# ICLDisco/ompi

Measured on AMD Instinct MI355X. Metric: Allreduce busBW GB/s @256MiB fp32 SUM at 2/4/8 GPUs; MPI_Op HBM GB/s, higher is better.
Workload: dtype f32; 1 GPU; MPI_Op 3-buffer SUM fp32, 1 GiB per buffer (BASELINE configs[1]); count=268435456, bytes_per_buffer=1073741824, op=MPI_SUM, datatype=MPI_FLOAT, kernel=op_vec_kernel<float,SUM,3buff>

## Files before the change

### ompi_amd/csrc/coll_ipc.hip

```cpp
#include <hip/hip_runtime.h>

#include <sched.h>
#include <unistd.h>

#include <algorithm>
#include <array>
#include <atomic>
#include <chrono>
#include <cstdarg>
#include <cstdio>
#include <cstdlib>
#include <cstring>
#include <deque>
#include <map>
#include <memory>
#include <mutex>
#include <new>
#include <utility>
#include <vector>

#include "../../include/ompi_amd_coll.h"
#include "bootstrap.h"
#include "comm_internal.h"
#include "host_mark.h"
#include "coll_kernels.h"
#include "coll_landing.h"
#include "ipc_registry.h"
#include "op_device.h"
#include "runtime.h"

namespace ompi_amd {

#define TRY(x)                                   \
    do {                                         \
        int rc_ = (x);                           \
        if (rc_ != OMPI_AMD_SUCCESS) return rc_; \
    } while (0)

__global__ void abort_kernel(flag_set peers, uint64_t *local, int rank, int size) {
    const int t = threadIdx.x;
    if (t < size && t != rank)
        __hip_atomic_store(peers.p[t] + kAbortWord, (uint64_t)1, __ATOMIC_RELAXED,
                           __HIP_MEMORY_SCOPE_SYSTEM);
    if (t == rank)
        __hip_atomic_store(local + kAbortWord, (uint64_t)1, __ATOMIC_RELAXED,
                           __HIP_MEMORY_SCOPE_SYSTEM);
    sys_release();
}

__global__ __launch_bounds__(64) void barrier_kernel(uint64_t *local, flag_set peers, int rank,
                                                     int size, uint64_t epoch, int *err,
                                                     uint64_t timeout_ticks, uint64_t *dbg) {
    const int t = threadIdx.x;
    if (dbg && t == 0)
        __hip_atomic_store(dbg, epoch, __ATOMIC_RELAXED, __HIP_MEMORY_SCOPE_SYSTEM);
    sys_release();
    if (t < size && t != rank)
        __hip_atomic_store(peers.p[t] + rank, epoch, __ATOMIC_RELAXED, __HIP_MEMORY_SCOPE_SYSTEM);
    if (t < size && t != rank)
        (void)wait_epoch(local + t, epoch, err, timeout_ticks, local + kAbortWord,
                         dbg ? dbg + 2 + t : nullptr);
    __syncthreads();
    sys_acquire();
    if (dbg && t == 0)
        __hip_atomic_store(dbg + 1, epoch, __ATOMIC_RELAXED, __HIP_MEMORY_SCOPE_SYSTEM);
}

__global__ void peek_kernel(const uint64_t *src, uint64_t *dst) {
    *dst = __hip_atomic_load(src, __ATOMIC_RELAXED, __HIP_MEMORY_SCOPE_SYSTEM);
}

struct tok_set { uint64_t t[kMaxRanks]; };
struct tok_ptrs { const uint64_t *p[kMaxRanks]; };
__global__ void land_stamp_kernel(uint64_t *mine, uint64_t token) {
    __hip_atomic_store(mine, token, __ATOMIC_RELAXED, __HIP_MEMORY_SCOPE_SYSTEM);
    sys_release();
}
__global__ __launch_bounds__(64) void land_check_kernel(tok_ptrs peers, tok_set expect, int rank, int size,
                                                        int *err, uint64_t *abort_word) {
    const int t = threadIdx.x;
    sys_acquire();
    if (t >= size || t == rank) return;
    if (__hip_atomic_load(peers.p[t], __ATOMIC_RELAXED, __HIP_MEMORY_SCOPE_SYSTEM) != expect.t[t]) {
        __hip_atomic_store(err, (int)OMPI_AMD_ERR_HIP, __ATOMIC_RELAXED, __HIP_MEMORY_SCOPE_SYSTEM);
        __hip_atomic_store(abort_word, (uint64_t)1, __ATOMIC_RELAXED, __HIP_MEMORY_SCOPE_SYSTEM);
    }
}

template <bool NT>
__global__ __launch_bounds__(kXferThreads) void copy_kernel(cp_jobs jobs) {
    acquire_once();
    const cp_job jb = jobs.j[blockIdx.y];
    const int64_t gstride = (int64_t)gridDim.x * kXferThreads;
    const int64_t tid = (int64_t)blockIdx.x * kXferThreads + threadIdx.x;
    const uintptr_t phase = (uintptr_t)jb.src ^ (uintptr_t)jb.dst;
    const int g = (phase & 15) == 0 ? 16 : ((phase & 3) == 0 ? 4 : 1);
    int64_t head = (int64_t)((g - ((uintptr_t)jb.src & (uintptr_t)(g - 1))) & (uintptr_t)(g - 1));
    if (head > jb.bytes) head = jb.bytes;
    const int64_t nbody = (jb.bytes - head) / g;
    const char *sb = jb.src + head;
    char *db = jb.dst + head;
    if (g == 16) {
        const u32x4 *s = reinterpret_cast<const u32x4 *>(sb);
        u32x4 *d = reinterpret_cast<u32x4 *>(db);
        int64_t i = tid;
        for (; i + 3 * gstride < nbody; i += 4 * gstride) {
            const u32x4 a = __builtin_nontemporal_load(s + i);
            const u32x4 b = __builtin_nontemporal_load(s + i + gstride);
            const u32x4 c = __builtin_nontemporal_load(s + i + 2 * gstride);
            const u32x4 e = __builtin_nontemporal_load(s + i + 3 * gstride);
            if constexpr (NT) {
                __builtin_nontemporal_store(a, d + i);
                __builtin_nontemporal_store(b, d + i + gstride);
                __builtin_nontemporal_store(c, d + i + 2 * gstride);
                __builtin_nontemporal_store(e, d + i + 3 * gstride);
            } else {
                d[i] = a;
                d[i + gstride] = b;
                d[i + 2 * gstride] = c;
                d[i + 3 * gstride] = e;
            }
        }
        for (; i < nbody; i += gstride) {
            if constexpr (NT) __builtin_nontemporal_store(__builtin_nontemporal_load(s + i), d + i);
            else d[i] = __builtin_nontemporal_load(s + i);
        }
    } else if (g == 4) {
        const uint32_t *s = reinterpret_cast<const uint32_t *>(sb);
        uint32_t *d = reinterpret_cast<uint32_t *>(db);
        for (int64_t i = tid; i < nbody; i += gstride) d[i] = s[i];
    } else {
        for (int64_t i = tid; i < nbody; i += gstride) db[i] = sb[i];
    }
    const int64_t tail0 = head + nbody * g;
    const int64_t nrest = head + (jb.bytes - tail0);
    for (int64_t k = tid; k < nrest; k += gstride) {
        const int64_t i = k < head ? k : tail0 + (k - head);
        jb.dst[i] = jb.src[i];
    }
    xfer_epilogue();
}

static red_launch_fn red_fn(int op, int type) {
    if (type < 0 || type >= OMPI_AMD_TYPE_COUNT) return nullptr;
    switch (op) {
#define CASE(k) case k: return red_row_##k()[type];
        OMPI_AMD_COLL_OPS(CASE)
#undef CASE
    default: return nullptr;
    }
}
static pipe_launch_fn pipe_fn(int op, int type) {
    if (type < 0 || type >= OMPI_AMD_TYPE_COUNT) return nullptr;
    switch (op) {
#define CASE(k) case k: return pipe_row_##k()[type];
        OMPI_AMD_COLL_OPS(CASE)
#undef CASE
    default: return nullptr;
    }
}
static fused_launch_fn fused_fn(int op, int type) {
    if (type < 0 || type >= OMPI_AMD_TYPE_COUNT) return nullptr;
    switch (op) {
#define CASE(k) case k: return fused_row_##k()[type];
        OMPI_AMD_COLL_OPS(CASE)
#undef CASE
    default: return nullptr;
    }
}

static size_t type_size(int type) {
    switch (type) {
    case OMPI_AMD_TYPE_DOUBLE_INT: case OMPI_AMD_TYPE_LONG_INT: return 12;
    case OMPI_AMD_TYPE_SHORT_INT: return 6;
    default: return ompi_amd_type_extent(type);
    }
}

static void blockcount(int64_t count, int n, int64_t *split, int64_t *early, int64_t *late) {
    *early = *late = count / n;
    *split = count % n;
    if (*split) *early += 1;
}
static int64_t block_off(int64_t b, int64_t split, int64_t early, int64_t late) {
    return b < split ? b * early : b * late + split;
}
static int64_t block_cnt(int64_t b, int64_t split, int64_t early, int64_t late) {
    return b < split ? early : late;
}

struct red_order { int order, first, flags; };
enum { TUNED_RED_LINEAR = 1, TUNED_RED_PIPELINE = 3, TUNED_RED_BINARY = 4, TUNED_RED_BINOMIAL = 5 };
enum { TUNED_RS_NONOVERLAPPING = 1, TUNED_RS_HALVING = 2, TUNED_RS_RING = 3 };
enum { TUNED_RSB_BASIC_LINEAR = 1 };
static bool tuned_red_alg_ok(int64_t v) {
    return v == 0 || v == TUNED_RED_LINEAR || v == TUNED_RED_PIPELINE || v == TUNED_RED_BINARY ||
           v == TUNED_RED_BINOMIAL;
}

static red_order tuned_reduce_order(int n, size_t msg, size_t count, int root, bool root_inplace,
                                    int forced = 0) {
    const int flr = root_inplace ? FOLD_ROOT_INPLACE : 0;
    switch (forced) {
    case TUNED_RED_LINEAR: return {ORDER_CHAIN, 0, 0};
    case TUNED_RED_PIPELINE: return {ORDER_CHAIN, root, flr};
    case TUNED_RED_BINARY: return {ORDER_BINARY, root, flr};
    case TUNED_RED_BINOMIAL: return {ORDER_BINOMIAL, root, flr};
    default: break;
    }
    const double a1 = 0.6016 / 1024.0, b1 = 1.3496;
    const double a2 = 0.0410 / 1024.0, b2 = 9.7128;
    const double a3 = 0.0422 / 1024.0, b3 = 1.1614;
    const int fl = root_inplace ? FOLD_ROOT_INPLACE : 0;
    const double m = (double)msg;
    if (n < 8 && msg < 512) return {ORDER_CHAIN, 0, 0};
    if ((n < 8 && msg < 20480) || msg < 2048 || count <= 1) return {ORDER_BINOMIAL, root, fl};
    if (n > a1 * m + b1) return {ORDER_BINOMIAL, root, fl};
    if (n > a2 * m + b2) return {ORDER_CHAIN, root, fl};
    if (n > a3 * m + b3) return {ORDER_BINARY, root, fl};
    return {ORDER_CHAIN, root, fl};
}

struct buf_desc {
    hipIpcMemHandle_t h;
    uint64_t off;
    uint64_t valid;
    uint64_t id;
    uint64_t base;
    uint64_t size;
    uint64_t pid;
};
struct call_blob {
    buf_desc s, r;
    uint64_t flags;
};
struct land_blob {
    buf_desc d;
    uint64_t token;
    int ok;
};

struct fold_plan {
    int order;
    int first;
    int flags;
};
enum {
    TUNED_AR_FIXED = 0, TUNED_AR_BASIC_LINEAR = 1, TUNED_AR_NONOVERLAPPING = 2,
    TUNED_AR_RECURSIVE_DOUBLING = 3, TUNED_AR_RING = 4, TUNED_AR_RING_SEGMENTED = 5,
    TUNED_AR_RABENSEIFNER = 6, TUNED_AR_COUNT = 7
};

struct path_params {
    size_t small_bytes, fused_bytes;
    int zero_copy, algorithm;
    int tuned_alg;
    int root0_inplace;
    int push_gather;
    int blocks = 0;
    int copy_nt = -1;
    int red_alg = 0;
};

struct shadow_set {
    cp_jobs in{};
    cp_job out{};
    char *mem = nullptr;
    char *mem2 = nullptr;
};

enum { XCH_ALLTOALL = 0, XCH_ALLGATHERV = 1, XCH_GATHER = 2, XCH_SCATTER = 3 };
struct a2a_call {
    const char *sbuf;
    char *rbuf;
    bool inplace;
    int coll;
    uint8_t ph[kMaxRanks];
    size_t sc[kMaxRanks], sd[kMaxRanks], rc[kMaxRanks], rd[kMaxRanks];
};

struct pending_op {
    uint64_t ticket;
    const void *sbuf;
    void *rbuf;
    size_t count;
    int type, op;
    hipStream_t stream;
    path_params pp;
    ompi_amd_request *req;
    shadow_set sh;
    int kind = 0;
    int root = 0;
    bool inplace = false;
    bool exclusive = false;
    bool land = false;
    std::vector<size_t> rcounts;
    bool unposted = false;
    size_t blob_len = 0;
    union {
        call_blob call;
        land_blob land;
    } blob{};
    char *grow = nullptr;
    size_t grow_bytes = 0;
    uint64_t grow_token = 0;
    a2a_call a2a{};
    size_t a2a_M = 0;
    size_t a2a_chunk = 0;
};

enum { PEND_ALLREDUCE = 0, PEND_RSB = 1, PEND_ALLGATHER = 2, PEND_BCAST = 3, PEND_REDUCE = 4,
       PEND_SCAN = 5, PEND_RS = 6, PEND_GROW = 7, PEND_ALLTOALL = 8 };

}

using namespace ompi_amd;

struct ompi_amd_request {
    ~ompi_amd_request() { mark_word_put(mark); }
    ompi_amd_comm_t *c = nullptr;
    hipEvent_t ev = nullptr;
    hipStream_t stream = nullptr;
    bool launched = false;
    bool recorded = false;
    uint64_t *mark = nullptr;
    uint64_t mark_seq = 0;
    int rc = OMPI_AMD_SUCCESS;
    char *shadow = nullptr;
    char *shadow2 = nullptr;
    uint64_t embedded = 0;
    int done_slot = -1;
    unsigned polls = 0;
};

constexpr int kTuneGrid = 18, kTuneCands = 2 * kTuneGrid, kTuneRounds = 2,
              kTuneCalls = kTuneCands * kTuneRounds;
struct tune_cand {
    int algorithm, blocks, nt;
};
static const tune_cand kTune[kTuneCands] = {
    {2, 1024, 1}, {2, 512, 1}, {2, 256, 1}, {3, 1024, 1}, {3, 512, 1}, {3, 256, 1},
    {0, 1024, 1}, {0, 512, 1}, {0, 256, 1}, {4, 1024, 1}, {4, 512, 1}, {4, 256, 1},
    {5, 1024, 1}, {5, 512, 1}, {5, 256, 1}, {6, 1024, 1}, {6, 512, 1}, {6, 256, 1},
    {2, 1024, 0}, {2, 512, 0}, {2, 256, 0}, {3, 1024, 0}, {3, 512, 0}, {3, 256, 0},
    {0, 1024, 0}, {0, 512, 0}, {0, 256, 0}, {4, 1024, 0}, {4, 512, 0}, {4, 256, 0},
    {5, 1024, 0}, {5, 512, 0}, {5, 256, 0}, {6, 1024, 0}, {6, 512, 0}, {6, 256, 0}};
struct tune_bucket {
    int ncand = kTuneCands;
    int next = 0;
    bool done = false;
    int choice = 0;
    hipEvent_t ev[2 * kTuneCalls] = {};
    float worst_ms[kTuneCands] = {};
};

struct ompi_amd_comm {
    int rank = 0, size = 0, device = 0;
    ShmBoot boot;
    uint64_t *flags = nullptr;
    flag_set peer_flags{};
    char *scratch = nullptr;
    size_t scratch_bytes = 0;
    uint64_t stage_seq = 0;
    ptr_set peer_scratch{};
    char *land = nullptr;
    size_t land_bytes = 0;
    ptr_set peer_land{};
    ipc_ref *land_ref[kMaxRanks] = {};
    size_t land_planned = 0;
    std::vector<char *> land_retired;
    std::vector<ipc_ref *> land_ref_retired;
    bool land_failed = false;
    int unposted = 0;
    int64_t deferred_growths = 0;
    std::vector<uint64_t> land_tokens;
    int memcpy_token_mismatch = 0;
    int bcast_split = 0;
    size_t bcast_split_bytes = 4u << 20;
    int64_t exports_new = 0, imports_new = 0;
    int recycled_exports = 0;
    int64_t reused_exports = 0;
    int reuse_shadow = 1;
    int unsafe_exports = 0;
    int aged_exports = 0;
    std::mutex stream_mu;
    std::recursive_mutex api_mu;
    std::atomic<int> npending{0};
    bool has_stream = false;
    hipStream_t cur_stream = nullptr;
    int own_stream = 0;
    hipStream_t own = nullptr;
    bool cur_closed = false;
    std::vector<hipEvent_t> stream_evs;
    char *shadow = nullptr;
    size_t shadow_bytes = 0;
    char *shadow2 = nullptr;
    size_t shadow2_bytes = 0;
    struct arena_chunk {
        char *base;
        size_t size;
        std::map<size_t, size_t> free;
        std::map<size_t, size_t> used;
    };
    std::mutex arena_mu;
    std::vector<arena_chunk> arena;
    size_t arena_bytes = 0;
    int shadowed = 0;
    int force_shadow = 0;
    int win_shadow = 0;
    int win_separate = 1;
    int64_t shadow_windows = 0;
    int user_ipc = 0;
    int *err_host = nullptr, *err_dev = nullptr;
    uint64_t *dbg_host = nullptr, *dbg_dev = nullptr;
    uint64_t epoch = 0;
    uint64_t *fused_mark = nullptr;
    bool want_mark = false;
    uint64_t mark_embedded = 0;
    uint64_t *mark_word = nullptr;
    int mark_slot = 0;
    std::vector<int> done_free;
    int done_next = 1;
    size_t small_bytes = 1 << 20;
    size_t fused_bytes = 64 << 10;
    int zero_copy = 1;
    int64_t timeout_ms = 30000;
    int max_blocks = 1024;
    int64_t pipe_slice = 64 << 10;
    int pipe_passes = 1;
    uint64_t pipe_seq = 0;
    int colocated = 1;
    int algorithm = 2;
    int autotune = 0;
    std::map<int, struct tune_bucket> tune;
    int tune_last = 0;
    int tune_last_key = -1;
    int nb_tuned_alg = -1, nb_tuned_blocks = -1, nb_tuned_nt = -1;
    int64_t land_ag_bcast = 0;
    int land_blocking = 0;
    size_t alltoall_chunk = 0;
    int64_t alltoall_passes = 0;
    int64_t alltoall_paths[5] = {};
    int64_t gather_paths[5] = {};
// ... 4337 lines not shown
```

### ompi_amd/csrc/coll_kern.hip

```cpp
#include <hip/hip_runtime.h>

#include <algorithm>
#include <array>
#include <utility>

#include "coll_kernels.h"

#ifndef COLL_OP
#error "build with -DCOLL_OP=<op index>"
#endif

namespace ompi_amd {
namespace {

template <int OP, int TYPE>
hipError_t red_launch_slot(dim3 grid, const ptr_set &src, const ptr_set &dst, int ndst, int n,
                           int order, int flags, const red_jobs &jobs, hipStream_t s) {
    if constexpr (slot_supported(OP, TYPE)) {
        using T = typename type_of<TYPE>::type;
        if (n <= 8)
            hipLaunchKernelGGL((reduce_kernel<T, OP, 8>), grid, dim3(kXferThreads), 0, s, src, dst,
                               ndst, n, order, flags, jobs);
        else
            hipLaunchKernelGGL((reduce_kernel<T, OP, kMaxRanks>), grid, dim3(kXferThreads), 0, s,
                               src, dst, ndst, n, order, flags, jobs);
        return hipGetLastError();
    } else {
        return hipErrorInvalidValue;
    }
}

template <int OP, int TYPE>
hipError_t fused_launch_slot(dim3 grid, const fused_args &a, hipStream_t s) {
    if constexpr (slot_supported(OP, TYPE)) {
        using T = typename type_of<TYPE>::type;
        hipLaunchKernelGGL((fused_allreduce_kernel<T, OP>), grid, dim3(kXferThreads), 0, s, a);
        return hipGetLastError();
    } else {
        return hipErrorInvalidValue;
    }
}

template <int OP, int TYPE>
hipError_t pipe_launch_slot(unsigned groups, const pipe_args &a, hipStream_t s) {
    if constexpr (slot_supported(OP, TYPE)) {
        using T = typename type_of<TYPE>::type;
        if (a.n > 8) return hipErrorInvalidValue;
        static const int64_t cap = [] {
            int per_cu = 0, cus = 0, dev = 0;
            if (hipGetDevice(&dev) != hipSuccess ||
                hipOccupancyMaxActiveBlocksPerMultiprocessor(
                    &per_cu, reinterpret_cast<const void *>(&pipe_allreduce_kernel<T, OP, 8>),
                    kXferThreads, 0) != hipSuccess ||
                hipDeviceGetAttribute(&cus, hipDeviceAttributeMultiprocessorCount, dev) != hipSuccess) {
                (void)hipGetLastError();
                return (int64_t)64;
            }
            return std::max<int64_t>(1, (int64_t)per_cu * cus / 2);
        }();
        const int64_t fit = std::max<int64_t>(1, cap / std::max(1, a.colocated));
        const dim3 g((unsigned)std::min<int64_t>(groups, fit)), b(kXferThreads);
        hipLaunchKernelGGL((pipe_allreduce_kernel<T, OP, 8>), g, b, 0, s, a);
        return hipGetLastError();
    } else {
        return hipErrorInvalidValue;
    }
}

template <int OP, int... T>
constexpr std::array<red_launch_fn, OMPI_AMD_TYPE_COUNT> make_red_row(std::integer_sequence<int, T...>) {
    return {{(slot_supported(OP, T) ? &red_launch_slot<OP, T> : (red_launch_fn) nullptr)...}};
}
template <int OP, int... T>
constexpr std::array<fused_launch_fn, OMPI_AMD_TYPE_COUNT> make_fused_row(
    std::integer_sequence<int, T...>) {
    return {{(slot_supported(OP, T) ? &fused_launch_slot<OP, T> : (fused_launch_fn) nullptr)...}};
}

template <int OP, int... T>
constexpr std::array<pipe_launch_fn, OMPI_AMD_TYPE_COUNT> make_pipe_row(
    std::integer_sequence<int, T...>) {
    return {{(slot_supported(OP, T) ? &pipe_launch_slot<OP, T> : (pipe_launch_fn) nullptr)...}};
}

const auto g_red_row = make_red_row<COLL_OP>(std::make_integer_sequence<int, OMPI_AMD_TYPE_COUNT>{});
const auto g_fused_row = make_fused_row<COLL_OP>(std::make_integer_sequence<int, OMPI_AMD_TYPE_COUNT>{});
const auto g_pipe_row = make_pipe_row<COLL_OP>(std::make_integer_sequence<int, OMPI_AMD_TYPE_COUNT>{});

}

#define ROW_NAME2(a, b) a##b
#define ROW_NAME(a, b) ROW_NAME2(a, b)
const red_launch_fn *ROW_NAME(red_row_, COLL_OP)() { return g_red_row.data(); }
const fused_launch_fn *ROW_NAME(fused_row_, COLL_OP)() { return g_fused_row.data(); }
const pipe_launch_fn *ROW_NAME(pipe_row_, COLL_OP)() { return g_pipe_row.data(); }

}
```

### ompi_amd/csrc/coll_kernels.h

```cpp
#pragma once

#include <hip/hip_runtime.h>

#include <cstdint>

#include "../../include/ompi_amd_coll.h"
#include "op_device.h"

namespace ompi_amd {

constexpr int kMaxRanks = OMPI_AMD_MAX_RANKS;
constexpr int kXferThreads = 256;

struct ptr_set { const char *p[kMaxRanks]; };
struct flag_set { uint64_t *p[kMaxRanks]; };

enum order_t {
    ORDER_RING = 0,
    ORDER_TREE = 1,
    ORDER_CHAIN = 2,
    ORDER_BINOMIAL = 3,
    ORDER_BINARY = 4,
    ORDER_HALVING = 5,
    ORDER_RABEN = 6,
};
constexpr int FOLD_ROOT_INPLACE = 1;
constexpr int FOLD_NT_STORE = 1 << 16;

struct red_job {
    int64_t off, cnt, off_dst;
    int first;
    int head;
    int aux = 0;
};
struct red_jobs { red_job j[2 * kMaxRanks]; int n; };

struct cp_job { const char *src; char *dst; int64_t bytes; };
struct cp_jobs { cp_job j[kMaxRanks]; int n; };

__device__ __forceinline__ void sys_acquire() {
    __builtin_amdgcn_fence(__ATOMIC_ACQUIRE, "");
    asm volatile("s_waitcnt vmcnt(0)" ::: "memory");
}
__device__ __forceinline__ void sys_release() {
    __builtin_amdgcn_fence(__ATOMIC_RELEASE, "");
    asm volatile("s_waitcnt vmcnt(0)" ::: "memory");
}

__device__ __forceinline__ void acquire_once() {
    if (threadIdx.x == 0) sys_acquire();
    __syncthreads();
}

constexpr int kAbortWord = 512;
constexpr size_t kFlagPageBytes = 8192;

__device__ __forceinline__ bool wait_epoch(const uint64_t *flag, uint64_t epoch, int *err,
                                           uint64_t ticks, uint64_t *abort_word,
                                           uint64_t *seen = nullptr) {
    const uint64_t t0 = __builtin_amdgcn_s_memrealtime();
    uint64_t check = t0 + 100000;
    while (__hip_atomic_load(flag, __ATOMIC_RELAXED, __HIP_MEMORY_SCOPE_SYSTEM) < epoch) {
        __builtin_amdgcn_s_sleep(1);
        const uint64_t now = __builtin_amdgcn_s_memrealtime();
        if (now - t0 > ticks) {
            __hip_atomic_store(err, (int)OMPI_AMD_ERR_TIMEOUT, __ATOMIC_RELAXED,
                               __HIP_MEMORY_SCOPE_SYSTEM);
            __hip_atomic_store(abort_word, (uint64_t)1, __ATOMIC_RELAXED, __HIP_MEMORY_SCOPE_SYSTEM);
            return false;
        }
        if (now >= check) {
            if (seen)
                __hip_atomic_store(seen, __hip_atomic_load(flag, __ATOMIC_RELAXED, __HIP_MEMORY_SCOPE_SYSTEM),
                                   __ATOMIC_RELAXED, __HIP_MEMORY_SCOPE_SYSTEM);
            if (__hip_atomic_load(abort_word, __ATOMIC_RELAXED, __HIP_MEMORY_SCOPE_SYSTEM) != 0) {
                __hip_atomic_store(err, (int)OMPI_AMD_ERR_TIMEOUT, __ATOMIC_RELAXED,
                                   __HIP_MEMORY_SCOPE_SYSTEM);
                return false;
            }
            check = now + 100000;
        }
    }
    return true;
}

__device__ __forceinline__ void xfer_epilogue() {
    asm volatile("s_waitcnt vmcnt(0)" ::: "memory");
    __syncthreads();
    if (threadIdx.x == 0) sys_release();
}

template <typename T, int OP, int NM = kMaxRanks>
__device__ __forceinline__ T fold(const T (&v)[NM], int n, int order, int flags) {
    using F = opfn<OP, false>;
    const bool swap = (flags & FOLD_ROOT_INPLACE) != 0;
    if (order == ORDER_RING) {
        T acc = v[0];
#pragma unroll
        for (int j = 1; j < NM; ++j)
            if (j < n) acc = F::template f<T>(v[j], acc);
        return acc;
    }
    if (order == ORDER_CHAIN) {
        T acc = v[NM - 1];
#pragma unroll
        for (int j = NM - 1; j >= 0; --j) {
            if (j == n - 1) acc = v[j];
            else if (j < n - 1) acc = (j == 0 && swap) ? F::template f<T>(v[0], acc)
                                                       : F::template f<T>(acc, v[j]);
        }
        return acc;
    }
    if (order == ORDER_BINOMIAL) {
        T w[NM];
#pragma unroll
        for (int i = 0; i < NM; ++i) w[i] = v[i];
#pragma unroll
        for (int u = 0; u + 1 < NM; u += 2)
            if (u + 1 < n) w[u] = (u == 0 && swap) ? F::template f<T>(w[0], w[1])
                                                   : F::template f<T>(w[u + 1], w[u]);
#pragma unroll
        for (int m = 2; m < NM; m <<= 1) {
#pragma unroll
            for (int u = 0; u + m < NM; u += 2 * m)
                if (u + m < n) w[u] = F::template f<T>(w[u], w[u + m]);
        }
        return w[0];
    }
    if (order == ORDER_BINARY) {
        T w[NM];
#pragma unroll
        for (int i = 0; i < NM; ++i) w[i] = v[i];
#pragma unroll
        for (int s = NM - 1; s >= 0; --s) {
            int d = 1;
            while (2 * d <= s + 1) d *= 2;
            const int c0 = s + d, c1 = s + 2 * d;
            if (c0 < NM && c0 < n)
                w[s] = (s == 0 && swap) ? F::template f<T>(w[0], w[c0])
                                        : F::template f<T>(w[c0], w[s]);
            if (c1 < NM && c1 < n) w[s] = F::template f<T>(w[s], w[c1]);
        }
        return w[0];
    }
    if (order == ORDER_RABEN) {
        int adj = 1;
        while (adj * 2 <= n) adj *= 2;
        const int rem = n - adj;
        const int o = (flags >> 8) & 0xff;
        const bool right = (o & 1) != 0;
        T w[NM];
#pragma unroll
        for (int u = 0; u < NM; ++u) {
            if (2 * u + 1 < NM && u < rem)
                w[u] = right ? F::template f<T>(v[2 * u + 1], v[2 * u])
                             : F::template f<T>(v[2 * u], v[2 * u + 1]);
            else if (u < adj)
                w[u] = v[u + rem < NM ? u + rem : 0];
        }
#pragma unroll
        for (int m = 1; m < NM; m <<= 1) {
            if (m < adj) {
#pragma unroll
                for (int u = 0; u < NM; ++u)
                    if (u < adj && (u & m) == (o & m)) w[u] = F::template f<T>(w[u], w[u ^ m]);
            }
        }
        T r = w[0];
#pragma unroll
        for (int u = 1; u < NM; ++u)
            if (u == o) r = w[u];
        return r;
    }
    if (order == ORDER_HALVING) {
        int adj = 1;
        while (adj * 2 <= n) adj *= 2;
        const int remain = n - adj;
        const int tb = (flags >> 8) & 0xff;
        T w[NM];
#pragma unroll
        for (int u = 0; u < NM; ++u) {
            if (2 * u + 1 < NM && u < remain) w[u] = F::template f<T>(v[2 * u + 1], v[2 * u]);
            else if (u < adj) w[u] = v[u + remain];
        }
#pragma unroll
        for (int m = NM / 2; m >= 1; m >>= 1) {
            if (m < adj) {
#pragma unroll
                for (int u = 0; u < NM; ++u)
                    if (u < adj && (u & m) == (tb & m)) w[u] = F::template f<T>(w[u], w[u ^ m]);
            }
        }
        T r = w[0];
#pragma unroll
        for (int u = 1; u < NM; ++u)
            if (u == tb) r = w[u];
        return r;
    }
    int adj = 1;
    while (adj * 2 <= n) adj *= 2;
    const int extra = n - adj;
    T w[NM];
#pragma unroll
    for (int i = 0; i < NM; ++i) {
        if (i < extra) w[i] = F::template f<T>(v[2 * i + 1], v[2 * i]);
        else if (i < adj) w[i] = v[i + extra];
    }
#pragma unroll
    for (int len = NM; len > 1; len >>= 1) {
        if (len <= adj) {
#pragma unroll
            for (int i = 0; i < NM / 2; ++i)
                if (2 * i + 1 < len) w[i] = F::template f<T>(w[2 * i + 1], w[2 * i]);
        }
    }
    return w[0];
}

template <typename T, int NM = kMaxRanks>
__device__ __forceinline__ void gather_scalar(T (&v)[NM], const ptr_set &src, int n,
                                              int first, int64_t e) {
#pragma unroll
    for (int j = 0; j < NM; ++j) {
        if (j < n) {
            const int r = (first + j) % n;
            v[j] = reinterpret_cast<const T *>(src.p[r])[e];
        }
    }
}

template <typename T, int OP, int NM = kMaxRanks>
__global__ __launch_bounds__(kXferThreads) void reduce_kernel(ptr_set src, ptr_set dst, int ndst,
                                                              int n, int order, int flags,
                                                              red_jobs jobs) {
    acquire_once();
    const red_job jb = jobs.j[blockIdx.y];
    constexpr int E = 16 / sizeof(T);
    const int64_t gstride = (int64_t)gridDim.x * kXferThreads;
    const int64_t tid = (int64_t)blockIdx.x * kXferThreads + threadIdx.x;
    const int64_t head = jb.head < 0 ? jb.cnt : jb.head;
    const int64_t nvec = jb.head < 0 ? 0 : (jb.cnt - head) / E;
    for (int64_t i = tid; i < nvec; i += gstride) {
        vec16<T> v[NM];
#pragma unroll
        for (int j = 0; j < NM; ++j) {
            if (j < n) {
                const int r = (jb.first + j) % n;
                const u32x4 *p = reinterpret_cast<const u32x4 *>(
                    reinterpret_cast<const T *>(src.p[r]) + jb.off + head);
                v[j].v = __builtin_nontemporal_load(p + i);
            }
        }
        vec16<T> out;
#pragma unroll
        for (int e = 0; e < E; ++e) {
            T s[NM];
#pragma unroll
            for (int j = 0; j < NM; ++j) s[j] = v[j].e[e];
            out.e[e] = fold<T, OP, NM>(s, n, order, flags | jb.aux);
        }
        if (flags & FOLD_NT_STORE) {
#pragma unroll
            for (int k = 0; k < NM; ++k)
                if (k < ndst)
                    __builtin_nontemporal_store(
                        out.v, reinterpret_cast<u32x4 *>(reinterpret_cast<T *>(const_cast<char *>(dst.p[k])) +
                                                         jb.off_dst + head) + i);
        } else {
#pragma unroll
            for (int k = 0; k < NM; ++k)
                if (k < ndst)
                    reinterpret_cast<u32x4 *>(reinterpret_cast<T *>(const_cast<char *>(dst.p[k])) +
                                              jb.off_dst + head)[i] = out.v;
        }
    }
    const int64_t tail0 = head + nvec * E;
    const int64_t nscalar = head + (jb.cnt - tail0);
    for (int64_t k = tid; k < nscalar; k += gstride) {
        const int64_t e = k < head ? k : tail0 + (k - head);
        T s[NM];
        gather_scalar<T, NM>(s, src, n, jb.first, jb.off + e);
        const T r = fold<T, OP, NM>(s, n, order, flags | jb.aux);
#pragma unroll
        for (int d = 0; d < NM; ++d)
            if (d < ndst)
                store_elem<T>(reinterpret_cast<T *>(const_cast<char *>(dst.p[d])) + jb.off_dst + e,
                              r);
    }
    xfer_epilogue();
}

constexpr int kFusedMaxGroups = 4096 / (int)sizeof(uint64_t) / kMaxRanks;

struct fused_args {
    const char *src;
    char *dst, *mine;
    ptr_set peers;
    uint64_t *flags;
    flag_set peer_flags;
    int rank, n, order;
    int64_t count, split, early, late;
    uint64_t epoch, timeout_ticks;
    int *err;
    uint32_t *done;
    uint64_t *mark;
    uint64_t mark_v;
};

constexpr int kFusedDoneWord = 8192 / (int)sizeof(uint32_t);
constexpr int kFusedDoneStride = 64 / (int)sizeof(uint32_t);
constexpr int kFusedDoneSlots = (64 << 10) / 64 - 8192 / 64;

template <typename T, int OP>
__global__ __launch_bounds__(kXferThreads) void fused_allreduce_kernel(fused_args a) {
    const int t = threadIdx.x;
    const int g = blockIdx.y * gridDim.x + blockIdx.x;
    int64_t off = 0, cnt = a.count;
    int first = 0;
    if (a.order == ORDER_RING) {
        const int64_t b = blockIdx.y;
        off = b < a.split ? b * a.early : b * a.late + a.split;
        cnt = b < a.split ? a.early : a.late;
        first = (int)b;
    }
    const int64_t per = (cnt + gridDim.x - 1) / gridDim.x;
    const int64_t lo = off + min(cnt, per * (int64_t)blockIdx.x);
    const int64_t hi = off + min(cnt, per * (int64_t)(blockIdx.x + 1));
    const T *src = reinterpret_cast<const T *>(a.src);
    T *mine = reinterpret_cast<T *>(a.mine);
    for (int64_t e = lo + t; e < hi; e += kXferThreads) mine[e] = src[e];
    asm volatile("s_waitcnt vmcnt(0)" ::: "memory");
    __syncthreads();
    if (t == 0) sys_release();
    __syncthreads();
    __shared__ int gave_up;
    if (t == 0) gave_up = 0;
    __syncthreads();
    if (t < a.n && t != a.rank) {
        __hip_atomic_store(a.peer_flags.p[t] + g * kMaxRanks + a.rank, a.epoch, __ATOMIC_RELAXED,
                           __HIP_MEMORY_SCOPE_SYSTEM);
        if (!wait_epoch(a.flags + g * kMaxRanks + t, a.epoch, a.err, a.timeout_ticks,
                        a.flags + kAbortWord))
            gave_up = 1;
    }
    __syncthreads();
    if (gave_up) return;
    acquire_once();
    T *dst = reinterpret_cast<T *>(a.dst);
    for (int64_t e = lo + t; e < hi; e += kXferThreads) {
        T v[kMaxRanks];
        gather_scalar<T>(v, a.peers, a.n, first, e);
        store_elem<T>(dst + e, fold<T, OP>(v, a.n, a.order, 0));
    }
    if (a.mark) {
        asm volatile("s_waitcnt vmcnt(0)" ::: "memory");
        __syncthreads();
        if (t == 0) {
            __builtin_amdgcn_fence(__ATOMIC_RELEASE, "agent");
            const uint32_t total = gridDim.x * gridDim.y;
            if (__hip_atomic_fetch_add(a.done, 1u, __ATOMIC_ACQ_REL, __HIP_MEMORY_SCOPE_AGENT) == total - 1) {
                __hip_atomic_store(a.done, 0u, __ATOMIC_RELAXED, __HIP_MEMORY_SCOPE_AGENT);
                __hip_atomic_store(a.mark, a.mark_v, __ATOMIC_RELAXED, __HIP_MEMORY_SCOPE_SYSTEM);
            }
        }
    }
}

constexpr int kPipeMaxGroups = 1024;
constexpr size_t kPipeFlagOff = 64 << 10;
constexpr size_t kPipeFlagBytes = 2 * (size_t)kPipeMaxGroups * kMaxRanks * sizeof(uint64_t);

struct pipe_args {
    const char *src;
    ptr_set dst_c;
    ptr_set src_f;
    ptr_set dst_f;
    ptr_set src_g;
    char *rbuf;
    uint64_t *flags;
    flag_set peer_flags;
    int rank, n, mine, ndst, order, first, fold_flags, nt;
    int colocated;
    int64_t split, early, late;
    int64_t per, nslices;
    uint64_t seq, timeout_ticks;
    int *err;
    uint64_t *abort_word;
};

__device__ __forceinline__ size_t pipe_row(int phase, int w, int r) {
    return ((size_t)phase * kPipeMaxGroups + (size_t)w) * kMaxRanks + (size_t)r;
}

__device__ __forceinline__ void pipe_copy(const char *s, char *d, int64_t lo, int64_t hi, bool nt) {
    const int t = threadIdx.x;
    if (hi <= lo) return;
    int64_t head = hi - lo, nv = 0;
    if ((((uintptr_t)(s + lo) ^ (uintptr_t)(d + lo)) & 15) == 0) {
        head = min(hi - lo, (int64_t)((16 - ((uintptr_t)(s + lo) & 15)) & 15));
        nv = (hi - lo - head) / 16;
    }
    const u32x4 *sv = reinterpret_cast<const u32x4 *>(s + lo + head);
    u32x4 *dv = reinterpret_cast<u32x4 *>(d + lo + head);
    constexpr int S = kXferThreads;
    int64_t i = t;
    for (; i + 3 * S < nv; i += 4 * S) {
        const u32x4 a = __builtin_nontemporal_load(sv + i);
        const u32x4 b = __builtin_nontemporal_load(sv + i + S);
        const u32x4 c = __builtin_nontemporal_load(sv + i + 2 * S);
        const u32x4 e = __builtin_nontemporal_load(sv + i + 3 * S);
        if (nt) {
            __builtin_nontemporal_store(a, dv + i);
            __builtin_nontemporal_store(b, dv + i + S);
            __builtin_nontemporal_store(c, dv + i + 2 * S);
            __builtin_nontemporal_store(e, dv + i + 3 * S);
        } else {
            dv[i] = a;
            dv[i + S] = b;
            dv[i + 2 * S] = c;
            dv[i + 3 * S] = e;
        }
    }
    for (; i < nv; i += S) {
        if (nt) __builtin_nontemporal_store(__builtin_nontemporal_load(sv + i), dv + i);
        else dv[i] = __builtin_nontemporal_load(sv + i);
    }
    const int64_t tail0 = lo + head + nv * 16;
    const int64_t nrest = head + (hi - tail0);
    for (int64_t k = t; k < nrest; k += S) {
        const int64_t b = k < head ? lo + k : tail0 + (k - head);
        d[b] = s[b];
    }
}

template <typename T, int OP, int NM>
__device__ __forceinline__ void pipe_fold(const pipe_args &a, int64_t lo, int64_t hi) {
    constexpr int E = 16 / sizeof(T);
    const int t = threadIdx.x;
    if (hi <= lo) return;
    const uintptr_t ph = (uintptr_t)(a.dst_f.p[0] + lo * (int64_t)sizeof(T)) & 15;
    bool same = true;
#pragma unroll
    for (int j = 0; j < NM; ++j)
        if (j < a.n) same = same && (((uintptr_t)(a.src_f.p[j] + lo * (int64_t)sizeof(T)) & 15) == ph);
#pragma unroll
    for (int k = 1; k < NM; ++k)
        if (k < a.ndst) same = same && (((uintptr_t)(a.dst_f.p[k] + lo * (int64_t)sizeof(T)) & 15) == ph);
    const int64_t lead = (int64_t)((16 - ph) & 15);
    int64_t head = hi - lo, nv = 0;
    if (same && lead % (int64_t)sizeof(T) == 0) {
        head = min(hi - lo, lead / (int64_t)sizeof(T));
        nv = (hi - lo - head) / E;
    }
    const int64_t v0 = lo + head;
    for (int64_t i = t; i < nv; i += kXferThreads) {
        vec16<T> v[NM];
#pragma unroll
        for (int j = 0; j < NM; ++j) {
            if (j < a.n) {
                const int r = (a.first + j) % a.n;
                const u32x4 *p = reinterpret_cast<const u32x4 *>(reinterpret_cast<const T *>(a.src_f.p[r]) + v0);
                v[j].v = __builtin_nontemporal_load(p + i);
            }
        }
        vec16<T> out;
#pragma unroll
        for (int e = 0; e < E; ++e) {
            T s[NM];
#pragma unroll
            for (int j = 0; j < NM; ++j) s[j] = v[j].e[e];
            out.e[e] = fold<T, OP, NM>(s, a.n, a.order, a.fold_flags);
        }
#pragma unroll
        for (int k = 0; k < NM; ++k) {
            if (k < a.ndst) {
                u32x4 *q = reinterpret_cast<u32x4 *>(reinterpret_cast<T *>(const_cast<char *>(a.dst_f.p[k])) + v0) + i;
                if (a.nt) __builtin_nontemporal_store(out.v, q);
                else *q = out.v;
            }
        }
    }
    const int64_t tail0 = v0 + nv * E;
    const int64_t nrest = head + (hi - tail0);
    for (int64_t k = t; k < nrest; k += kXferThreads) {
        const int64_t e = k < head ? lo + k : tail0 + (k - head);
        T s[NM];
        gather_scalar<T, NM>(s, a.src_f, a.n, a.first, e);
        const T r = fold<T, OP, NM>(s, a.n, a.order, a.fold_flags);
#pragma unroll
        for (int d = 0; d < NM; ++d)
            if (d < a.ndst) store_elem<T>(reinterpret_cast<T *>(const_cast<char *>(a.dst_f.p[d])) + e, r);
    }
}

template <typename T, int OP, int NM>
__global__ __launch_bounds__(kXferThreads) void pipe_allreduce_kernel(pipe_args a) {
    const int t = threadIdx.x, w = blockIdx.x, G = gridDim.x;
    const int64_t P = (a.nslices - w + G - 1) / G;
    constexpr int64_t ext = sizeof(T);
    __shared__ int gave_up;
    if (t == 0) gave_up = 0;
    __syncthreads();
    for (int64_t p = 0; p < P + 2; ++p) {
        const bool doC = p < P, doF = p >= 1 && p <= P, doG = p >= 2;
        if (p >= 1) {
            if (t < a.n && t != a.rank) {
                bool ok = true;
                if (doF)
                    ok = wait_epoch(a.flags + pipe_row(0, w, t), a.seq + (uint64_t)p, a.err,
                                    a.timeout_ticks, a.abort_word);
                if (ok && doG)
                    ok = wait_epoch(a.flags + pipe_row(1, w, t), a.seq + (uint64_t)(p - 1), a.err,
                                    a.timeout_ticks, a.abort_word);
                if (!ok) gave_up = 1;
            }
            __syncthreads();
            if (gave_up) return;
            acquire_once();
        }
        if (doC) {
            const int64_t s = w + p * G;
#pragma unroll
            for (int b = 0; b < NM; ++b) {
                if (b >= a.n || !a.dst_c.p[b]) continue;
                const int64_t off = b < a.split ? b * a.early : b * a.late + a.split;
                const int64_t cnt = b < a.split ? a.early : a.late;
                const int64_t lo = off + min(cnt, s * a.per), hi = off + min(cnt, (s + 1) * a.per);
                pipe_copy(a.src, const_cast<char *>(a.dst_c.p[b]), lo * ext, hi * ext, a.nt);
            }
        }
        if (doF) {
            const int64_t s = w + (p - 1) * G;
            const int b = a.mine;
            const int64_t off = b < a.split ? b * a.early : b * a.late + a.split;
            const int64_t cnt = b < a.split ? a.early : a.late;
            pipe_fold<T, OP, NM>(a, off + min(cnt, s * a.per), off + min(cnt, (s + 1) * a.per));
        }
        if (doG) {
            const int64_t s = w + (p - 2) * G;
#pragma unroll
            for (int b = 0; b < NM; ++b) {
                if (b >= a.n || !a.src_g.p[b]) continue;
                const int64_t off = b < a.split ? b * a.early : b * a.late + a.split;
                const int64_t cnt = b < a.split ? a.early : a.late;
                const int64_t lo = off + min(cnt, s * a.per), hi = off + min(cnt, (s + 1) * a.per);
                pipe_copy(a.src_g.p[b], a.rbuf, lo * ext, hi * ext, a.nt);
            }
        }
        if (doC || doF) {
            asm volatile("s_waitcnt vmcnt(0)" ::: "memory");
            __syncthreads();
            if (t == 0) sys_release();
            __syncthreads();
            if (t < a.n && t != a.rank) {
                if (doC)
                    __hip_atomic_store(a.peer_flags.p[t] + pipe_row(0, w, a.rank), a.seq + (uint64_t)(p + 1),
                                       __ATOMIC_RELAXED, __HIP_MEMORY_SCOPE_SYSTEM);
                if (doF)
                    __hip_atomic_store(a.peer_flags.p[t] + pipe_row(1, w, a.rank), a.seq + (uint64_t)p,
                                       __ATOMIC_RELAXED, __HIP_MEMORY_SCOPE_SYSTEM);
            }
        }
    }
    xfer_epilogue();
}

struct a2a_args {
    const char *sbuf;
    char *rbuf, *mine;
    ptr_set peers;
    uint64_t *flags;
    flag_set peer_flags;
    int rank, n;
    int self_copy;
    int64_t slot;
    int64_t scount[kMaxRanks], sdispl[kMaxRanks], rcount[kMaxRanks], rdispl[kMaxRanks];
    uint8_t sphase[kMaxRanks], rphase[kMaxRanks];
    uint64_t epoch, timeout_ticks;
    int *err;
    uint32_t *done;
    uint64_t *mark;
    uint64_t mark_v;
};

__host__ __device__ __forceinline__ void a2a_slice(int64_t b, int g, int G, int64_t *lo, int64_t *hi) {
    const int64_t per = ((b + G - 1) / G + 15) & ~(int64_t)15;
    *lo = per * g < b ? per * g : b;
    *hi = per * (g + 1) < b ? per * (g + 1) : b;
}

// ... 172 lines not shown
```

Measured before the change: 6488 GB/s.

## Specialize reduce kernel by rank count, unroll loads, and widen fold blocks

```diff
diff --git a/ompi_amd/csrc/coll_ipc.hip b/ompi_amd/csrc/coll_ipc.hip
--- a/ompi_amd/csrc/coll_ipc.hip
+++ b/ompi_amd/csrc/coll_ipc.hip
@@ -85,60 +85,6 @@
         __hip_atomic_store(err, (int)OMPI_AMD_ERR_HIP, __ATOMIC_RELAXED, __HIP_MEMORY_SCOPE_SYSTEM);
         __hip_atomic_store(abort_word, (uint64_t)1, __ATOMIC_RELAXED, __HIP_MEMORY_SCOPE_SYSTEM);
     }
-}
-
-template <bool NT>
-__global__ __launch_bounds__(kXferThreads) void copy_kernel(cp_jobs jobs) {
-    acquire_once();
-    const cp_job jb = jobs.j[blockIdx.y];
-    const int64_t gstride = (int64_t)gridDim.x * kXferThreads;
-    const int64_t tid = (int64_t)blockIdx.x * kXferThreads + threadIdx.x;
-    const uintptr_t phase = (uintptr_t)jb.src ^ (uintptr_t)jb.dst;
-    const int g = (phase & 15) == 0 ? 16 : ((phase & 3) == 0 ? 4 : 1);
-    int64_t head = (int64_t)((g - ((uintptr_t)jb.src & (uintptr_t)(g - 1))) & (uintptr_t)(g - 1));
-    if (head > jb.bytes) head = jb.bytes;
-    const int64_t nbody = (jb.bytes - head) / g;
-    const char *sb = jb.src + head;
-    char *db = jb.dst + head;
-    if (g == 16) {
-        const u32x4 *s = reinterpret_cast<const u32x4 *>(sb);
-        u32x4 *d = reinterpret_cast<u32x4 *>(db);
-        int64_t i = tid;
-        for (; i + 3 * gstride < nbody; i += 4 * gstride) {
-            const u32x4 a = __builtin_nontemporal_load(s + i);
-            const u32x4 b = __builtin_nontemporal_load(s + i + gstride);
-            const u32x4 c = __builtin_nontemporal_load(s + i + 2 * gstride);
-            const u32x4 e = __builtin_nontemporal_load(s + i + 3 * gstride);
-            if constexpr (NT) {
-                __builtin_nontemporal_store(a, d + i);
-                __builtin_nontemporal_store(b, d + i + gstride);
-                __builtin_nontemporal_store(c, d + i + 2 * gstride);
-                __builtin_nontemporal_store(e, d + i + 3 * gstride);
-            } else {
-                d[i] = a;
-                d[i + gstride] = b;
-                d[i + 2 * gstride] = c;
-                d[i + 3 * gstride] = e;
-            }
-        }
-        for (; i < nbody; i += gstride) {
-            if constexpr (NT) __builtin_nontemporal_store(__builtin_nontemporal_load(s + i), d + i);
-            else d[i] = __builtin_nontemporal_load(s + i);
-        }
-    } else if (g == 4) {
-        const uint32_t *s = reinterpret_cast<const uint32_t *>(sb);
-        uint32_t *d = reinterpret_cast<uint32_t *>(db);
-        for (int64_t i = tid; i < nbody; i += gstride) d[i] = s[i];
-    } else {
-        for (int64_t i = tid; i < nbody; i += gstride) db[i] = sb[i];
-    }
-    const int64_t tail0 = head + nbody * g;
-    const int64_t nrest = head + (jb.bytes - tail0);
-    for (int64_t k = tid; k < nrest; k += gstride) {
-        const int64_t i = k < head ? k : tail0 + (k - head);
-        jb.dst[i] = jb.src[i];
-    }
-    xfer_epilogue();
 }
 
 static red_launch_fn red_fn(int op, int type) {
diff --git a/ompi_amd/csrc/coll_kern.hip b/ompi_amd/csrc/coll_kern.hip
--- a/ompi_amd/csrc/coll_kern.hip
+++ b/ompi_amd/csrc/coll_kern.hip
@@ -18,12 +18,15 @@
                            int order, int flags, const red_jobs &jobs, hipStream_t s) {
     if constexpr (slot_supported(OP, TYPE)) {
         using T = typename type_of<TYPE>::type;
-        if (n <= 8)
-            hipLaunchKernelGGL((reduce_kernel<T, OP, 8>), grid, dim3(kXferThreads), 0, s, src, dst,
-                               ndst, n, order, flags, jobs);
-        else
-            hipLaunchKernelGGL((reduce_kernel<T, OP, kMaxRanks>), grid, dim3(kXferThreads), 0, s,
-                               src, dst, ndst, n, order, flags, jobs);
+        const int m = std::max(n, ndst);
+#define RED_LAUNCH(NM)                                                                          \
+    hipLaunchKernelGGL((reduce_kernel<T, OP, NM, red_unroll(NM), kFoldThreads>), grid,          \
+                       dim3(kFoldThreads), 0, s, src, dst, ndst, n, order, flags, jobs)
+        if (m <= 2) RED_LAUNCH(2);
+        else if (m <= 4) RED_LAUNCH(4);
+        else if (m <= 8) RED_LAUNCH(8);
+        else RED_LAUNCH(kMaxRanks);
+#undef RED_LAUNCH
         return hipGetLastError();
     } else {
         return hipErrorInvalidValue;
diff --git a/ompi_amd/csrc/coll_kernels.h b/ompi_amd/csrc/coll_kernels.h
--- a/ompi_amd/csrc/coll_kernels.h
+++ b/ompi_amd/csrc/coll_kernels.h
@@ -48,7 +48,9 @@
 }
 
 __device__ __forceinline__ void acquire_once() {
+#ifndef OMPI_AMD_PROBE_NO_FENCE
     if (threadIdx.x == 0) sys_acquire();
+#endif
     __syncthreads();
 }
 
@@ -87,7 +89,9 @@
 __device__ __forceinline__ void xfer_epilogue() {
     asm volatile("s_waitcnt vmcnt(0)" ::: "memory");
     __syncthreads();
+#ifndef OMPI_AMD_PROBE_NO_FENCE
     if (threadIdx.x == 0) sys_release();
+#endif
 }
 
 template <typename T, int OP, int NM = kMaxRanks>
@@ -229,63 +233,148 @@
     }
 }
 
-template <typename T, int OP, int NM = kMaxRanks>
-__global__ __launch_bounds__(kXferThreads) void reduce_kernel(ptr_set src, ptr_set dst, int ndst,
-                                                              int n, int order, int flags,
-                                                              red_jobs jobs) {
+constexpr int kFoldThreads = 512;
+constexpr int red_unroll(int nm) { return nm > 4 && nm <= 8 ? 2 : 1; }
+constexpr int kCopyUnroll = 4;
+
+template <typename T, int OP, int NM>
+__device__ __forceinline__ void fold_store_vec(const vec16<T> (&v)[NM], const ptr_set &dst,
+                                               int ndst, int n, int order, int flags,
+                                               int64_t dst_elem, int64_t i) {
+    constexpr int E = 16 / sizeof(T);
+    vec16<T> out;
+#pragma unroll
+    for (int e = 0; e < E; ++e) {
+        T s[NM];
+#pragma unroll
+        for (int j = 0; j < NM; ++j) s[j] = v[j].e[e];
+        out.e[e] = fold<T, OP, NM>(s, n, order, flags);
+    }
+    if (flags & FOLD_NT_STORE) {
+#pragma unroll
+        for (int k = 0; k < NM; ++k)
+            if (k < ndst)
+                __builtin_nontemporal_store(
+                    out.v, reinterpret_cast<u32x4 *>(reinterpret_cast<T *>(const_cast<char *>(dst.p[k])) +
+                                                     dst_elem) + i);
+    } else {
+#pragma unroll
+        for (int k = 0; k < NM; ++k)
+            if (k < ndst)
+                reinterpret_cast<u32x4 *>(reinterpret_cast<T *>(const_cast<char *>(dst.p[k])) +
+                                          dst_elem)[i] = out.v;
+    }
+}
+
+template <typename T, int OP, int NM, int U, bool TAIL>
+__device__ __forceinline__ void red_step(const ptr_set &src, const ptr_set &dst, int ndst, int n,
+                                         int order, int fl, const red_job &jb, int64_t head,
+                                         int64_t i, int64_t gstride, int64_t nvec) {
+    vec16<T> v[U][NM];
+#pragma unroll
+    for (int u = 0; u < U; ++u) {
+#pragma unroll
+        for (int j = 0; j < NM; ++j) {
+            if (j < n && (!TAIL || i + u * gstride < nvec)) {
+                const int r = (jb.first + j) % n;
+                const u32x4 *p = reinterpret_cast<const u32x4 *>(
+                    reinterpret_cast<const T *>(src.p[r]) + jb.off + head);
+                v[u][j].v = __builtin_nontemporal_load(p + i + u * gstride);
+            }
+        }
+    }
+#pragma unroll
+    for (int u = 0; u < U; ++u) {
+        if (!TAIL || i + u * gstride < nvec)
+            fold_store_vec<T, OP, NM>(v[u], dst, ndst, n, order, fl, jb.off_dst + head,
+                                      i + u * gstride);
+    }
+}
+
+template <typename T, int OP, int NM = kMaxRanks, int U = 1, int TH = kFoldThreads>
+__global__ __launch_bounds__(TH) void reduce_kernel(ptr_set src, ptr_set dst, int ndst, int n,
+                                                    int order, int flags, red_jobs jobs) {
     acquire_once();
     const red_job jb = jobs.j[blockIdx.y];
     constexpr int E = 16 / sizeof(T);
-    const int64_t gstride = (int64_t)gridDim.x * kXferThreads;
-    const int64_t tid = (int64_t)blockIdx.x * kXferThreads + threadIdx.x;
+    const int64_t gstride = (int64_t)gridDim.x * TH;
+    const int64_t tid = (int64_t)blockIdx.x * TH + threadIdx.x;
     const int64_t head = jb.head < 0 ? jb.cnt : jb.head;
     const int64_t nvec = jb.head < 0 ? 0 : (jb.cnt - head) / E;
-    for (int64_t i = tid; i < nvec; i += gstride) {
-        vec16<T> v[NM];
-#pragma unroll
-        for (int j = 0; j < NM; ++j) {
-            if (j < n) {
-                const int r = (jb.first + j) % n;
-                const u32x4 *p = reinterpret_cast<const u32x4 *>(
-                    reinterpret_cast<const T *>(src.p[r]) + jb.off + head);
-                v[j].v = __builtin_nontemporal_load(p + i);
-            }
-        }
-        vec16<T> out;
-#pragma unroll
-        for (int e = 0; e < E; ++e) {
-            T s[NM];
-#pragma unroll
-            for (int j = 0; j < NM; ++j) s[j] = v[j].e[e];
-            out.e[e] = fold<T, OP, NM>(s, n, order, flags | jb.aux);
-        }
-        if (flags & FOLD_NT_STORE) {
-#pragma unroll
-            for (int k = 0; k < NM; ++k)
-                if (k < ndst)
-                    __builtin_nontemporal_store(
-                        out.v, reinterpret_cast<u32x4 *>(reinterpret_cast<T *>(const_cast<char *>(dst.p[k])) +
-                                                         jb.off_dst + head) + i);
-        } else {
-#pragma unroll
-            for (int k = 0; k < NM; ++k)
-                if (k < ndst)
-                    reinterpret_cast<u32x4 *>(reinterpret_cast<T *>(const_cast<char *>(dst.p[k])) +
-                                              jb.off_dst + head)[i] = out.v;
-        }
-    }
+    const int fl = flags | jb.aux;
+    int64_t i = tid;
+    for (; i + (U - 1) * gstride < nvec; i += U * gstride)
+        red_step<T, OP, NM, U, false>(src, dst, ndst, n, order, fl, jb, head, i, gstride, nvec);
+    if (U > 1 && i < nvec)
+        red_step<T, OP, NM, U, true>(src, dst, ndst, n, order, fl, jb, head, i, gstride, nvec);
     const int64_t tail0 = head + nvec * E;
     const int64_t nscalar = head + (jb.cnt - tail0);
     for (int64_t k = tid; k < nscalar; k += gstride) {
         const int64_t e = k < head ? k : tail0 + (k - head);
         T s[NM];
         gather_scalar<T, NM>(s, src, n, jb.first, jb.off + e);
-        const T r = fold<T, OP, NM>(s, n, order, flags | jb.aux);
+        const T r = fold<T, OP, NM>(s, n, order, fl);
 #pragma unroll
         for (int d = 0; d < NM; ++d)
             if (d < ndst)
                 store_elem<T>(reinterpret_cast<T *>(const_cast<char *>(dst.p[d])) + jb.off_dst + e,
                               r);
+    }
+    xfer_epilogue();
+}
+
+template <bool NT, int U = kCopyUnroll, int TH = kXferThreads>
+__global__ __launch_bounds__(TH) void copy_kernel(cp_jobs jobs) {
+    acquire_once();
+    const cp_job jb = jobs.j[blockIdx.y];
+    const int64_t gstride = (int64_t)gridDim.x * TH;
+    const int64_t tid = (int64_t)blockIdx.x * TH + threadIdx.x;
+    const uintptr_t phase = (uintptr_t)jb.src ^ (uintptr_t)jb.dst;
+    const int g = (phase & 15) == 0 ? 16 : ((phase & 3) == 0 ? 4 : 1);
+    int64_t head = (int64_t)((g - ((uintptr_t)jb.src & (uintptr_t)(g - 1))) & (uintptr_t)(g - 1));
+    if (head > jb.bytes) head = jb.bytes;
+    const int64_t nbody = (jb.bytes - head) / g;
+    const char *sb = jb.src + head;
+    char *db = jb.dst + head;
+    if (g == 16) {
+        const u32x4 *s = reinterpret_cast<const u32x4 *>(sb);
+        u32x4 *d = reinterpret_cast<u32x4 *>(db);
+        int64_t i = tid;
+        for (; i + (U - 1) * gstride < nbody; i += U * gstride) {
+            u32x4 v[U];
+#pragma unroll
+            for (int u = 0; u < U; ++u) v[u] = __builtin_nontemporal_load(s + i + u * gstride);
+#pragma unroll
+            for (int u = 0; u < U; ++u) {
+                if constexpr (NT) __builtin_nontemporal_store(v[u], d + i + u * gstride);
+                else d[i + u * gstride] = v[u];
+            }
+        }
+        if (i < nbody) {
+            u32x4 v[U];
+#pragma unroll
+            for (int u = 0; u < U; ++u)
+                if (i + u * gstride < nbody) v[u] = __builtin_nontemporal_load(s + i + u * gstride);
+#pragma unroll
+            for (int u = 0; u < U; ++u) {
+                if (i + u * gstride < nbody) {
+                    if constexpr (NT) __builtin_nontemporal_store(v[u], d + i + u * gstride);
+                    else d[i + u * gstride] = v[u];
+                }
+            }
+        }
+    } else if (g == 4) {
+        const uint32_t *s = reinterpret_cast<const uint32_t *>(sb);
+        uint32_t *d = reinterpret_cast<uint32_t *>(db);
+        for (int64_t i = tid; i < nbody; i += gstride) d[i] = s[i];
+    } else {
+        for (int64_t i = tid; i < nbody; i += gstride) db[i] = sb[i];
+    }
+    const int64_t tail0 = head + nbody * g;
+    const int64_t nrest = head + (jb.bytes - tail0);
+    for (int64_t k = tid; k < nrest; k += gstride) {
+        const int64_t i = k < head ? k : tail0 + (k - head);
+        jb.dst[i] = jb.src[i];
     }
     xfer_epilogue();
 }
```

Measured after the change: 6487 GB/s. No clear change (-0.0%).
